# esteinig/sketchy

Hardware: AMD Instinct MI355X
Metric: reads/sec streamed (s=10000,k=16,40k-genome ref) (higher is better)
Workload: dtype u64

## Files before the change

### sketchy_amd/csrc/skx_capi.hip

```cpp
#include <dlfcn.h>
#include <hip/hip_runtime.h>
#include <rccl/rccl.h>

#include <unistd.h>

#include <algorithm>
#include <atomic>
#include <chrono>
#include <cmath>
#include <condition_variable>
#include <cstdarg>
#include <cstdio>
#include <cstdlib>
#include <cstring>
#include <mutex>
#include <string>
#include <thread>
#include <unordered_map>
#include <vector>

#include "sketchy_hip.h"
#include "skx_common.hpp"
#include "skx_kernels.hpp"

// ... 914 lines not shown
    bool back_pending[2] = {false, false};
    hipEvent_t ev_pslot[3] = {nullptr, nullptr, nullptr};
    bool pslot_pending[3] = {false, false, false};
    int pslot = 0;
    hipEvent_t ev_pairq[2] = {nullptr, nullptr};
    bool pairq_pending[2] = {false, false};
    bool packed = false;
    u32 top_k = 0, max_reads = 0, sk_stride = 0;
    u64 max_bases = 0;
    u32 pcap = 0;
    u32 qcap = 0;
    u64* d_qd = nullptr;
    u32 *d_qrow = nullptr, *d_sslot = nullptr, *d_qinfo = nullptr, *d_qloc = nullptr, *d_cls_bsum = nullptr;
    u32* d_nd_hs = nullptr;
    u32* h_lcount = nullptr;
    u32 lcount_seq = 0, lcount_seen = 0, lcount_floor = 0;
    u32* h_nq_sink = nullptr;
    u32* h_nd = nullptr;
    u32 *d_rowcnt = nullptr;
    u32 *d_gain = nullptr;
    u32 *d_gain_s = nullptr;
    u32 *d_candslot = nullptr;
    u32 *d_candmask = nullptr;
    uint2 *d_lrow = nullptr;
    u32 *d_nlrow = nullptr, *d_gain_l = nullptr, *d_cbase = nullptr, *d_cwl = nullptr, *d_ncwl = nullptr;
    u64 *d_cw = nullptr;
    u64 *d_inb = nullptr, *d_hit = nullptr;
    skx::LongRows long_rows() const { return skx::LongRows{d_lrow, d_nlrow, qcap + 128, d_inb, ref->n_lw}; }
    bool use_pat = false;
    u32 *d_hist = nullptr, *d_nprow = nullptr;
    u64* d_pcw = nullptr;
    u32 npat_pad = 0;
    skx::PatRows pat_rows() const { return skx::PatRows{d_hist, npat_pad, d_gain_l, d_nprow}; }
    skx::RareIndex rare_index() const {
        skx::RareIndex ri = ref->rare_index();
        if (!use_pat) { ri.prec = nullptr; ri.n_pat = 0; }
        if (!static_dense) { ri.qs = nullptr; ri.n_sd = 0; }
        return ri;
    }
    u32 *d_cbad = nullptr, *d_nqc = nullptr;
    u32 *d_spc_g0 = nullptr, *d_spc_grp = nullptr;
    u32 n_pad_c = 0, n_grp_c = 0, cand_seq = 0;
    struct PassSet {
        u64 *tab = nullptr;
        u32 *cand = nullptr;
        u64 *tabc = nullptr;
        u32 *ncand = nullptr;
        u32 *mode = nullptr, *any_full = nullptr, *nqc_total = nullptr;
        u64 *mc = nullptr;
        u64 *mqc = nullptr;
        u64 *rowany_c = nullptr;
        u32 *grp_any_c = nullptr;
        u32 *smap = nullptr;
        u32 *pair_qc = nullptr;
        u32 *nd = nullptr;
        u32 *h_pub = nullptr;
    } ps[2];
    struct PassChains {
        bool pending = false, ranked = false, has_cand = false, update_table = false, forced_full = false, legacy = false;
        SubPass subs[kGroupMax];
        int n_sub = 0, b = 0, slot = 0;
        u32 P = 0, nq_rows = 0, seq = 0;
        u64 nq_est = 0;
    } pcq[2];
    int pc_head = 0, pc_n = 0;
    bool hint_all_overflow = false;
    u32 hint_seq = 0;
    u32 passes_since_fresh = 0;
    bool fresh_table = true;
    u32 legacy_run = 0;
    u64 batches_compact = 0, batches_full = 0;
    bool have_split_hint = false;
    double nd_frac = 1.0;
    u32 qcap_max = 0;
    bool qcap_auto = false;
    u64 qrows_grown = 0;
    u32 coalesce = 1;
    u32 rpass = 0;
    u64 reads_total = 0;
    uint8_t* d_bases = nullptr;
    u64* d_offsets = nullptr;
    u64* d_sk = nullptr;
    u32 *d_len = nullptr, *d_cnt = nullptr, *d_poff = nullptr;
    bool side_ready[kSides] = {};
    u64* sd_sk[kSides] = {};
    u64 pool_cap[kSides] = {};
    u32 pool_fixed = 0;
    u64* sd_rows[kSides] = {};
    u32 cur_stride = 0;
    u32 cur_pool_cap = 0, cur_pool_fixed = 0;
    u32 *sd_len[kSides] = {}, *sd_cnt[kSides] = {}, *sd_poff[kSides] = {}, *sd_big[kSides] = {};
// ... 130 lines not shown
static void free_side(skx_stream* st, int i);
static void free_lane(skx_stream* st, int i);
static void free_call(CallOut& d) {
    void* ptrs[] = {d.sp, d.idx, d.sum, d.codes, d.n_events, d.ev_read, d.ev_sp, d.ev_idx, d.ev_sum, d.ev_codes};
    for (void* q : ptrs) (void)hipFree(q);
    d = CallOut{};
}
static void stream_free(skx_stream* st) {
    if (!st) return;
    (void)hipSetDevice(st->device);
    if (st->hs0) (void)hipStreamSynchronize(st->hs0);
    if (st->hs1) (void)hipStreamSynchronize(st->hs1);
    if (st->hs) (void)hipStreamSynchronize(st->hs);
    if (st->hs2) (void)hipStreamSynchronize(st->hs2);
    for (int i = 1; i < skx_stream::kRankLanes; ++i)
        if (st->lane[i].s) (void)hipStreamSynchronize(st->lane[i].s);
    for (int i = 0; i < kSides; ++i) (void)hipFree(st->sd_rows[i]);
    void* ptrs[] = {st->d_bases, st->d_offsets, st->d_pair_h[0], st->d_pair_h[1],
                    st->d_q[0], st->d_q[1], st->d_pair_r[0], st->d_pair_r[1], st->d_pair_q[0], st->d_pair_q[1],
                    st->d_poff_pass[0], st->d_poff_pass[1], st->d_poff_pass[2], st->d_pair_r[2], st->d_nq[0], st->d_nq[1], st->d_win[0], st->d_win[1], st->d_m, st->d_mint, st->d_mq[0], st->d_mq[1],
                    st->d_topk_idx, st->d_topk_sum, st->d_cons, st->d_ev.n_events, st->d_ev.ev_read, st->d_ev.ev_idx, st->d_ev.ev_sum, st->d_ev.ev_codes, st->d_tab_tmp, st->d_rank_idx, st->d_rank_sum, st->d_bsum, st->d_grp_any[0],
                    st->d_grp_any[1], st->d_hbuf, st->d_wb[0], st->d_wb[1], st->d_rowany[0], st->d_rowany[1], st->d_mqext,
                    st->d_qd, st->d_qrow, st->d_sslot, st->d_qinfo, st->d_qloc, st->d_cls_bsum, st->d_nd_hs,
                    st->d_rowcnt, st->d_gain, st->d_gain_s, st->d_candslot, st->d_candmask, st->d_lrow, st->d_nlrow, st->d_gain_l, st->d_cbase, st->d_cwl, st->d_ncwl, st->d_cw, st->d_cbad, st->d_nqc, st->d_spc_g0, st->d_spc_grp, st->d_inb, st->d_hit, st->d_hist, st->d_nprow, st->d_pcw, st->d_ms[0], st->d_ms[1], st->d_mdirty_s};
    for (auto& q : st->ps) {
        for (void* x : {(void*)q.tab, (void*)q.cand, (void*)q.tabc, (void*)q.ncand, (void*)q.mode, (void*)q.any_full, (void*)q.nqc_total, (void*)q.mc, (void*)q.mqc,
                        (void*)q.rowany_c, (void*)q.grp_any_c, (void*)q.smap, (void*)q.pair_qc, (void*)q.nd}) (void)hipFree(x);
        if (q.h_pub) (void)hipHostFree(q.h_pub);
    }
    for (auto& t : st->d_tab) (void)hipFree(t);
    for (int i = 0; i < skx_stream::kRankLanes; ++i) free_lane(st, i);
    for (int i = 1; i < skx_stream::kRankLanes; ++i)
        if (st->own_lane_stream && st->lane[i].s) (void)hipStreamDestroy(st->lane[i].s);
    for (void* p : ptrs) (void)hipFree(p);
    for (void* p : {(void*)st->d_seen, (void*)st->d_cov_pad, (void*)st->d_cov_out, (void*)st->d_cov_list, (void*)st->d_cov_ridx,
                    (void*)st->d_cov_wide, (void*)st->d_cov_rsum}) (void)hipFree(p);
    if (st->h_poff) (void)hipHostFree(st->h_poff);
    if (st->h_offsets) (void)hipHostFree(st->h_offsets);
    if (st->h_nq) (void)hipHostFree(st->h_nq);
    if (st->h_nd) (void)hipHostFree(st->h_nd);
    if (st->h_nq_sink) (void)hipHostFree(st->h_nq_sink);
    if (st->h_lcount) (void)hipHostFree(st->h_lcount);
    if (st->h_chk_base) (void)hipHostFree(st->h_chk_base);
    for (int i = 0; i < kSides; ++i) {
        free_side(st, i);
        if (st->ev_main[i]) (void)hipEventDestroy(st->ev_main[i]);
    }
// ... 398 lines not shown
    memset(st->h_nd, 0, 4 * 4);
    SCHK(hipHostMalloc((void**)&st->h_nq_sink, 4 * 4, hipHostMallocCoherent));
    SCHK(hipHostMalloc((void**)&st->h_lcount, 4 * 4, hipHostMallocCoherent));
    memset(st->h_lcount, 0, 4 * 4);
    SCHK(hipMalloc(&st->d_nd_hs, 64));
    SCHK(hipMemset(st->d_nd_hs, 0, 64));
    if (ref->d_kt_key) {
        SCHK(hipMalloc(&st->d_qd, (size_t)st->pcap * 8));
        SCHK(hipMalloc(&st->d_qrow, (size_t)st->pcap * 4));
        SCHK(hipMalloc(&st->d_sslot, (size_t)st->pcap * 8));
        SCHK(hipMalloc(&st->d_qinfo, (size_t)st->pcap * 4));
        SCHK(hipMalloc(&st->d_qloc, (size_t)st->pcap * 4));
        SCHK(hipMalloc(&st->d_cls_bsum, ((size_t)st->pcap / 1024 + 2) * 4));
    }
    {
        const u32 nb = skx::kPassBatchesMax, cap = skx::kCandCap, rows_c = skx::kCandRows;
        st->n_pad_c = n_sp * cap;
        st->n_grp_c = st->n_pad_c / (skx::kRankWords * 64);
        SCHK(hipMalloc(&st->d_rowcnt, (size_t)nb * ((size_t)st->qcap + 128) * 4));
        SCHK(hipMalloc(&st->d_gain, (size_t)nb * n_pad * 4));
        if (ref->d_kt_key) SCHK(hipMalloc(&st->d_gain_s, (size_t)nb * n_pad * 4 * skx::gain_sparse_stride()));
        SCHK(hipMalloc(&st->d_candslot, (size_t)nb * n_pad * 4));
        SCHK(hipMalloc(&st->d_candmask, (size_t)n_pad * 4));
        if (ref->d_mlong) {
            SCHK(hipMalloc(&st->d_lrow, (size_t)nb * ((size_t)st->qcap + 128) * 8));
            SCHK(hipMalloc(&st->d_nlrow, skx::pass_counter_bytes()));
            SCHK(hipMalloc(&st->d_gain_l, (size_t)nb * n_pad * 4));
            SCHK(hipMalloc(&st->d_cw, (size_t)nb * (n_pad / 64) * 8));
            SCHK(hipMalloc(&st->d_cbase, (size_t)nb * (n_pad / 64) * 4));
            SCHK(hipMalloc(&st->d_cwl, (size_t)nb * st->n_pad_c * 4));
            SCHK(hipMalloc(&st->d_ncwl, 64));
            if (ref->d_mlongT) {
                SCHK(hipMalloc(&st->d_inb, (size_t)nb * ref->n_lw * 8));
                SCHK(hipMalloc(&st->d_hit, (size_t)nb * ref->n_lw * 8));
            }
            if (ref->d_prec && ref->n_pat && st->n_grp_c * skx::kRankWords <= skx::pat_words_max()) {
                st->use_pat = true;
                st->npat_pad = (ref->n_pat + 63u) & ~63u;
                SCHK(hipMalloc(&st->d_hist, (size_t)nb * st->npat_pad * 4));
                SCHK(hipMalloc(&st->d_nprow, skx::pass_counter_bytes()));
                SCHK(hipMalloc(&st->d_pcw, (size_t)nb * ref->n_pat * st->n_grp_c * skx::kRankWords * 8));
            }
        }
        SCHK(hipMalloc(&st->d_cbad, 64));
        SCHK(hipMalloc(&st->d_nqc, skx::pass_counter_bytes()));
        std::vector<u32> g0c(n_sp), grpc(st->n_grp_c);
// ... 296 lines not shown
    HIPCHK(hipMemsetAsync(d_mdirty, 0, 4, hs));
    SKX_MARK("pass: memset mdirty", 0);
    auto wait_back = [&]() -> int {
        if (st->back_pending[b]) { HIPCHK(hipStreamWaitEvent(hs, st->ev_back[b], 0)); st->back_pending[b] = false; }
        HIPCHK(hipMemcpyAsync(ps.nd, d_nd, 16, hipMemcpyDeviceToDevice, hs));
        HIPCHK(hipMemsetAsync(d_grp_any, 0, (size_t)n_grp_all * 4, hs));
        if (P > 0) {
            skx::launch_pair_q(hs, st->d_pair_h[b], P, d_q, d_nq, d_pair_q, split_dict ? st->d_qrow : nullptr, st->d_bbase, st->d_btot, ref->max_ref);
            HIPCHK(hipGetLastError());
        }
        HIPCHK(hipEventRecord(st->ev_pairq[b], hs));
        st->pairq_pending[b] = true;
        return SKX_OK;
    };
    bool ranked = false, all_forced = false, all_ranked = true;
    for (int i = 0; i < n_sub; ++i) {
        const bool r = st->top_k && subs[i].d_topk_idx && subs[i].d_topk_sum;
        ranked = ranked || r; all_ranked = all_ranked && r && !subs[i].d_shared && !subs[i].d_counts;
    }
    const u32* only_if = nullptr;
    u32 seq = 0;
    static const int legacy_env = skx::knob("SKX_TABLE_LEGACY") ? atoi(skx::knob("SKX_TABLE_LEGACY")) : 1 << 30;
    static const int cand_env0 = skx::knob("SKX_CAND") ? atoi(skx::knob("SKX_CAND")) : 1;
    const bool fresh_overflow = st->fresh_table && ref->max_species > skx::kCandCap && st->top_k <= 1;
    const bool second_blind = st->passes_since_fresh == 1 && !((int)(st->lcount_seen - st->lcount_floor) > 0);
    const bool legacy = update_table && all_ranked && cand_env0 && legacy_env > 0 &&
                        (fresh_overflow || (st->hint_all_overflow && !second_blind && (int)st->legacy_run < legacy_env));
    st->legacy_run = legacy ? st->legacy_run + 1 : 0;
    if (update_table) { st->passes_since_fresh = st->fresh_table ? 1 : st->passes_since_fresh + 1; st->fresh_table = false; }
    const bool long_rows = split_dict && ref->d_mlong != nullptr;
    static const int tail_env = skx::knob("SKX_TAIL_SCALE") ? atoi(skx::knob("SKX_TAIL_SCALE")) : 8;
    const u32 walk_scale = st->tail_pass ? (u32)std::max(1, tail_env) : 1u;
    skx::PassBatches pbt;
    pbt.n = (u32)n_sub;
    for (int i = 0; i < n_sub; ++i) pbt.p_off[i] = subs[i].p_off;
    pbt.p_off[n_sub] = P;
    auto rare_gains = [&](hipStream_t on) -> int {
        const skx::RareIndex ri = st->rare_index();
        const skx::LongRows lrows = st->long_rows();
        const skx::PatRows prows = st->pat_rows();
        skx::launch_gain_sparse(on, d_nd, q_bound, st->d_rowcnt, qstride, (u32)n_sub, n_pad, st->d_gain_s, st->d_sslot, ri, long_rows ? &lrows : nullptr, walk_scale,
                                (long_rows && st->use_pat) ? &prows : nullptr);
        if (long_rows) skx::launch_gain_long(on, lrows, ri, d_nd, st->d_rowcnt, qstride, (u32)n_sub, n_pad, st->d_gain_l, walk_scale);
        if (long_rows && st->use_pat)
            skx::launch_gain_dense(on, ri.pm, nullptr, n_pad, ri.d_npat, ri.n_pat, st->d_hist, st->npat_pad, (u32)n_sub, st->d_gain_l);
        HIPCHK(hipGetLastError());
        return SKX_OK;
    };
    auto row_counts = [&]() -> int {
        HIPCHK(hipMemset2DAsync(st->d_rowcnt, (size_t)qstride * 4, 0, (size_t)nq_rows * 4, (size_t)n_sub, hs));
        skx::launch_pass_hist(hs, d_pair_q, pbt, st->d_rowcnt, qstride);
        if (split_dict) HIPCHK(hipMemsetAsync(st->d_gain_s, 0, (size_t)n_sub * n_pad * 4 * skx::gain_sparse_stride(), hs));
// ... 61 lines not shown
        const u64* m_int = split ? st->d_mint : nullptr;
        HIPCHK(hipMemsetAsync(st->d_gain, 0, (size_t)n_sub * n_pad * 4, hs));
        if (P > 0) {
            SKXCHK(row_counts());
            skx::launch_gain_dense(hs, d_m, m_int, n_pad, d_nd, sdm ? ref->n_sd : q_bound, st->d_rowcnt, qstride, (u32)n_sub, st->d_gain,
                                   (sdm && ref->n_species > 1) ? ref->d_segw : nullptr, ref->d_grp_sp);
            if (split_dict) SKXCHK(rare_gains(hs));
        }
        skx::launch_pass_tables(hs, st->d_cum, st->d_gain, (split_dict && P > 0) ? st->d_gain_s : nullptr,
                                (long_rows && P > 0) ? st->d_gain_l : nullptr, (u32)n_sub, n_pad, ps.tab);
        st->d_cum = ps.tab + (size_t)n_sub * n_pad;
        static const int cand_env = skx::knob("SKX_CAND") ? atoi(skx::knob("SKX_CAND")) : 1;
        static const int hint_env = skx::knob("SKX_CAND_HINT") ? atoi(skx::knob("SKX_CAND_HINT")) : 1;
        (void)hint_env;
        all_forced = !cand_env;
        u32 force_full = all_forced ? 0xFFu : 0u;
        for (int i = 0; i < n_sub; ++i) if (subs[i].d_shared || subs[i].d_counts) force_full |= 1u << i;
        HIPCHK(hipMemsetAsync(st->d_cbad, 0, 64, hs));
        HIPCHK(hipMemsetAsync(st->d_nqc, 0, skx::pass_counter_bytes(), hs));
        const bool pat_rows = st->use_pat && long_rows && ranked && P > 0 && !all_forced;
        if (pat_rows) skx::launch_pat_nqc_init(hs, st->d_nqc, st->npat_pad);
        if (ranked) {
            HIPCHK(hipMemsetAsync(st->d_candmask, 0, (size_t)n_pad * 4, hs));
            skx::launch_cand_select(hs, ps.tab, n_pad, spc, (u32)n_sub, st->top_k, cap, ps.cand, st->d_candslot, ps.tabc, ps.ncand, st->d_cbad,
                                    st->d_candmask);
            HIPCHK(hipMemsetAsync(ps.grp_any_c, 0, (size_t)n_sub * st->n_grp_c * 4, hs));
            if (split_dict && P > 0 && !all_forced) {
                HIPCHK(hipMemsetAsync(ps.mqc, 0, (size_t)n_sub * st->n_grp_c * rows_c * skx::kRankWords * 8, hs));
                HIPCHK(hipMemsetAsync(ps.rowany_c, 0, (size_t)n_sub * st->n_grp_c * (rows_c / 64) * 8, hs));
                HIPCHK(hipMemset2DAsync(ps.smap, (size_t)qstride * 4, 0, (size_t)nq_rows * 4, (size_t)n_sub, hs));
                skx::launch_cand_sparse(hs, st->d_sslot, d_nd, q_bound, st->rare_index(), st->d_candmask, st->d_candslot, n_pad, st->d_cbad, (u32)n_sub, st->d_nqc,
                                        ps.smap, qstride, ps.mqc, (size_t)st->n_grp_c * rows_c * skx::kRankWords, rows_c, ps.rowany_c,
                                        st->n_grp_c * (rows_c / 64), ps.grp_any_c, st->n_grp_c, walk_scale);
                if (long_rows) {
                    const u32 n_gw = n_pad / 64;
                    HIPCHK(hipMemsetAsync(st->d_cw, 0, (size_t)n_sub * n_gw * 8, hs));
                    HIPCHK(hipMemsetAsync(st->d_cbase, 0xFF, (size_t)n_sub * n_gw * 4, hs));
                    HIPCHK(hipMemsetAsync(st->d_ncwl, 0, 64, hs));
                    skx::launch_cand_words(hs, ps.cand, st->n_pad_c, (u32)n_sub, n_gw, st->d_cw, st->d_cbase, st->d_cwl, st->d_ncwl);
                    if (st->d_hit) skx::launch_cand_hit(hs, ps.cand, st->n_pad_c, (u32)n_sub, st->d_cbad, st->rare_index(), st->d_inb, st->d_hit);
                    skx::launch_cand_long(hs, st->long_rows(), st->rare_index(), d_nd, st->d_cw, st->d_cbase, st->d_cwl, st->d_ncwl, st->n_pad_c,
                                          st->d_cbad, (u32)n_sub, st->d_nqc, ps.smap, qstride, ps.mqc, (size_t)st->n_grp_c * rows_c * skx::kRankWords,
                                          rows_c, ps.rowany_c, st->n_grp_c * (rows_c / 64), ps.grp_any_c, st->n_grp_c, walk_scale, st->d_hit);
                }
                if (pat_rows) {
                    const skx::RareIndex ri = st->rare_index();
                    skx::launch_cand_pat_rows(hs, ri, d_nd, st->d_candmask, st->d_candslot, n_pad, st->d_cbad, (u32)n_sub, st->d_pcw, ps.mqc,
                                              (size_t)st->n_grp_c * rows_c * skx::kRankWords, rows_c, ps.rowany_c, st->n_grp_c * (rows_c / 64), ps.grp_any_c,
// ... 373 lines not shown
    if (call) sb.call = *call;
    sb.ra = ra; sb.rb = rb; sb.p_off = 0; sb.P = P; sb.p_base = p_base; sb.d_topk_idx = d_topk_idx; sb.d_topk_sum = d_topk_sum;
    sb.d_shared = d_shared; sb.d_counts = d_counts; sb.side = st->side;
    sb.d_poff = st->d_poff_pass[st->pslot];
    return run_pass_multi(st, &sb, 1, update_table, inserted, q_rows);
}

template <class F>
static int for_each_pass(skx_stream* st, u32 n_reads, u32 max_pass_reads, F fn) {
    const u32 cap = std::max<u32>(1u, std::min<u32>(st->rpass, max_pass_reads));
    const u32 pair_cap = std::min(st->pcap, st->qhash_cap());
    u32 ra = 0;
    while (ra < n_reads) {
        u32 rb = ra;
        while (rb < n_reads && rb - ra < cap && st->h_poff[rb + 1] - st->h_poff[ra] <= pair_cap) ++rb;
        if (rb == ra) return fail(SKX_ERR_CAPACITY, "read %u alone has %u candidate hashes > pass capacity %u", ra,
                                  st->h_poff[ra + 1] - st->h_poff[ra], pair_cap);
        SKXCHK(fn(ra, rb, st->h_poff[ra], st->h_poff[rb] - st->h_poff[ra]));
        ra = rb;
    }
    return SKX_OK;
}

static int wait_published(skx_stream* st, const PendingBatch& pb) {
    volatile u32* pub = st->h_chk_base + 16 * pb.side;
    hipStream_t hs = st->hs1;
    for (u64 spins = 1; pub[15] != pb.seq; ++spins) {
        if ((spins & 0xFFF) == 0) {
            const hipError_t e = hipStreamQuery(hs);
            if (e == hipSuccess) {
                if (pub[15] == pb.seq) break;
                HIPCHK(hipStreamSynchronize(hs));
                if (pub[15] != pb.seq) return fail(SKX_ERR_HIP, "publish kernel finished without raising its sequence number");
            } else if (e != hipErrorNotReady) {
                return fail(SKX_ERR_HIP, "stream failed while waiting for the batch summary: %s", hipGetErrorString(e));
            }
        }
    }
    return SKX_OK;
}
static const u64* batch_filter(const skx_ref* ref) {
    static const bool no_filter = skx::knob("SKX_NO_FILTER") != nullptr;
    return (ref->any && !no_filter) ? ref->d_filt : nullptr;
}
static int behind_the_sketch(skx_stream* st, int side) {
    if (st->hs1 == st->hs0) return SKX_OK;
    HIPCHK(hipEventRecord(st->ev_main[side], st->hs0));
    HIPCHK(hipStreamWaitEvent(st->hs1, st->ev_main[side], 0));
    return SKX_OK;
}
// ... 279 lines not shown
    }
    SKX_ACC(back);
#ifdef SKX_EXPERIMENTS
    g_ht.n += 1;
    if (skx::knob("SKX_HOST_TIMES") && (g_ht.n % 64) == 0)
        fprintf(stderr, "[skx host times] per batch over %llu: front %.1f us, wait for summary %.1f us, queue passes %.1f us\n",
                (unsigned long long)g_ht.n, g_ht.front / g_ht.n, g_ht.wait / g_ht.n, g_ht.back / g_ht.n);
#endif
    if (d_shared) (void)hipFree(d_shared);
    SKXCHK(pass_rc);
    st->reads_total += n_reads;
    return SKX_OK;
}

static int batch_back_group(skx_stream* st, PendingBatch* g, int n, PendingBatch* younger, int* n_done) {
    *n_done = 0;
    if (n == 1) {
        SKXCHK(batch_back(st, g[0], younger));
        *n_done = 1;
        return SKX_OK;
    }
    {
        SKX_T0();
        for (int i = 0; i < n; ++i) SKXCHK(wait_published(st, g[i]));
        SKX_ACC(wait);
    }
    bool fits = st->buf == g[0].spec_set && st->pslot == g[0].spec_slot;
    u64 pairs = 0;
    u32 P[kGroupMax];
    for (int i = 0; i < n; ++i) {
        const volatile u32* c = st->h_chk_base + 16 * g[i].side;
        fits = fits && !(c[0] | c[6] | c[7]);
        P[i] = c[8];
        pairs += P[i];
    }
    const u32 q_rows = (st->h_chk_base + 16 * g[n - 1].side)[10];
    const bool clean = fits;
    if (clean && q_rows != 0xFFFFFFFFu && q_rows > st->qhash_cap() && pairs <= st->pcap)
        SKXCHK(grow_query_rows(st, ((u64)q_rows + q_rows / 4) * std::max<u32>(1u, (st->coalesce + (u32)n - 1) / (u32)n)));
    fits = fits && pairs <= st->pcap && q_rows != 0xFFFFFFFFu && q_rows <= st->qhash_cap();
    u64 reads = 0;
    for (int i = 0; i < n; ++i) reads += g[i].n_reads;
    if (clean && q_rows != 0xFFFFFFFFu && reads) {
        st->ppr_est = (double)pairs / reads;
        st->qpr_est = (double)q_rows / reads;
    }
    if (clean && !fits) {
// ... 1738 lines not shown
```

### sketchy_amd/csrc/skx_kernels.hip

```cpp
#include <algorithm>
#include <cstdlib>
#include <mutex>
#include <type_traits>

#include "skx_common.hpp"
#include "skx_kernels.hpp"

#ifndef SKX_FEW_CANDS
#define SKX_FEW_CANDS 8
#endif
#ifndef SKX_SCAN_ROWS
#define SKX_SCAN_ROWS 8
#endif
#ifndef SKX_SCAN_OCC
#define SKX_SCAN_OCC 1
#endif
#ifndef SKX_SCAN_SPLIT_READS
#define SKX_SCAN_SPLIT_READS 1
#endif
#ifndef SKX_WALK_BLOCKS
#define SKX_WALK_BLOCKS 256
#endif
#ifndef SKX_GAIN_SPARSE_STRIDE
#define SKX_GAIN_SPARSE_STRIDE 16
// ... 4200 lines not shown
    return theta;
}
__global__ __launch_bounds__(1024) void cand_count_kernel(const u64* __restrict__ t0, const u64* __restrict__ t1, Species sp, u32 top_k,
                                                          u32* __restrict__ d_max, volatile u32* __restrict__ h_out, u32 seq) {
    __builtin_amdgcn_s_setprio(3);
    __shared__ u64 sh64[16];
    __shared__ u32 sh32[16];
    u32 worst = 0;
    for (u32 spi = 0; spi < sp.n_sp; ++spi) {
        const u32 g0 = sp.g0[spi], n = sp.n[spi];
        const u64 theta = species_theta(t0, g0, n, top_k, sh64, sh32);
        u32 c = 0;
        for (u32 g = g0 + threadIdx.x; g < g0 + n; g += 1024u) c += t1[g] >= theta ? 1u : 0u;
        worst = max(worst, block1024_sum_u32(c, sh32));
    }
    if (threadIdx.x == 0u) {
        (void)d_max;
        h_out[0] = worst;
        __threadfence_system();
        h_out[1] = seq;
        __threadfence_system();
    }
}
__global__ __launch_bounds__(1024) void cand_select_kernel(const u64* __restrict__ tab, u32 n_pad, Species sp, u32 top_k, u32 cap,
                                                           u32* __restrict__ cand, u32* __restrict__ candslot, u64* __restrict__ tabc,
                                                           u32* __restrict__ ncand, u32* __restrict__ bad, u32* __restrict__ candmask) {
    __builtin_amdgcn_s_setprio(3);
    __shared__ u64 sh64[16];
    __shared__ u32 sh32[16];
    __shared__ u32 wbase[17];
    const u32 b = blockIdx.x / sp.n_sp, spi = blockIdx.x % sp.n_sp, tid = threadIdx.x, lane = lane_id(), wv = tid >> 6;
    const u32 g0 = sp.g0[spi], n = sp.n[spi];
    const u32 g_end = spi + 1u < sp.n_sp ? sp.g0[spi + 1u] : n_pad;
    const u64* t0 = tab + (size_t)b * n_pad;
    const u64* t1 = t0 + n_pad;
    const u64 theta = species_theta(t0, g0, n, top_k, sh64, sh32);
    u32 base = 0;
    u32* my_cand = cand + (size_t)(b * sp.n_sp + spi) * cap;
    u64* my_tabc = tabc + (size_t)b * sp.n_sp * cap + (size_t)spi * cap;
    for (u32 c0 = g0; c0 < g_end; c0 += 1024u) {
        const u32 g = c0 + tid;
        const bool is = g < g0 + n && t1[g] >= theta;
        const u64 bal = __ballot(is);
        const u32 before = (u32)__popcll(bal & lanemask_lt()), wtot = (u32)__popcll(bal);
        __syncthreads();
        if (lane == 0u) wbase[wv] = wtot;
        __syncthreads();
        u32 wb = 0, tot = 0;
#pragma unroll
        for (u32 i = 0; i < 16u; ++i) { const u32 v = wbase[i]; wb += i < wv ? v : 0u; tot += v; }
        const u32 pos = base + wb + before;
        if (g < g_end) {
            u32 slot = kCandNone;
            if (is && pos < cap) { my_cand[pos] = g; my_tabc[pos] = t0[g]; slot = spi * cap + pos; atomicOr(&candmask[g], 1u << b); }
            candslot[(size_t)b * n_pad + g] = slot;
        }
        base += tot;
    }
    for (u32 i = min(base, cap) + tid; i < cap; i += 1024u) { my_cand[i] = kCandNone; my_tabc[i] = 0; }
    if (tid == 0u) {
        ncand[b * sp.n_sp + spi] = min(base, cap);
        if (base > cap) atomicOr(&bad[b], 1u);
    }
}
__global__ __launch_bounds__(256) void cand_gather_m_kernel(const u64* __restrict__ m_bits, const u64* __restrict__ m_int, u32 n_pad,
                                                            const u32* __restrict__ n_d,
                                                            const u32* __restrict__ cand, u32 n_pad_c, const u32* __restrict__ bad,
                                                            u64* __restrict__ mc, u32 words_c) {
    __builtin_amdgcn_s_setprio(2);
    const u32 b = blockIdx.z, w = blockIdx.y, c = blockIdx.x * 256u + threadIdx.x;
    if (bad[b] || w >= ((n_d[0] + 63u) >> 6) || c >= n_pad_c) return;
    const u32 g = cand[(size_t)b * n_pad_c + c];
    u64 x = 0;
    if (g != kCandNone) { x = m_bits[(size_t)w * n_pad + g]; if (m_int) x |= m_int[(size_t)w * n_pad + g]; }
    mc[((size_t)b * words_c + w) * n_pad_c + c] = x;
}
__global__ __launch_bounds__(256) void cand_sparse_kernel(const u32* __restrict__ sslot, const u32* __restrict__ n_d, RareIndex ri,
                                                          const u32* __restrict__ candmask, const u32* __restrict__ candslot, u32 n_pad,
                                                          u32* __restrict__ bad, u32 n_b, u32* __restrict__ nqc, u32* __restrict__ smap,
                                                          u32 smap_stride, u64* __restrict__ mqc, size_t mqc_stride, u32 rows_c,
                                                          u64* __restrict__ rowany_c, u32 rowany_stride, u32* __restrict__ grp_any_c,
                                                          u32 n_grp_c) {
    __builtin_amdgcn_s_setprio(2);
    __shared__ u64 pat[4][kPassBatchesMax][kPatWords];
    const u32 nd64 = n_d[2], ns = n_d[1], lane = lane_id();
    const u32 n_gw_c = n_grp_c * kRankWords;
    const u32 wave = blockIdx.x * 4u + (threadIdx.x >> 6), n_waves = gridDim.x * 4u;
    auto put = [&](u32 b, u32 crow, u32 slot) { atomicOr(&mqc[(size_t)b * mqc_stride + mq_index(slot >> 6, crow, rows_c)], 1ull << (slot & 63u)); };
    auto flag = [&](u32 b, u32 crow, u32 grp) {
        atomicOr(&rowany_c[(size_t)b * rowany_stride + (size_t)grp * (rows_c >> 6) + (crow >> 6)], 1ull << (crow & 63u));
        u32* ga = grp_any_c + (size_t)b * n_grp_c + grp;
        if (*ga == 0u) atomicOr(ga, 1u);
    };
    auto new_row = [&](u32 b, u32 sr) -> u32 {
        if (bad[b]) return kCandNone;
        const u32 crow = nd64 + atomicAdd(&nqc[b * kCtrStride], 1u);
        if (crow + 1u >= rows_c) { atomicOr(&bad[b], 2u); return kCandNone; }
        smap[(size_t)b * smap_stride + sr] = crow + 1u;
        return crow;
    };
    for (u32 r0 = wave * 64u; r0 < ns; r0 += n_waves * 64u) {
        const u32 sr = r0 + lane;
        u32 off = 0, np = 0;
        if (sr < ns) { const uint2 e = reinterpret_cast<const uint2*>(sslot)[sr]; off = e.x; np = e.y; }
        if (np & kLongFlag) np = 0;
        if (np && np <= 8u) {
            u32 crow[kPassBatchesMax];
#pragma unroll
            for (u32 b = 0; b < kPassBatchesMax; ++b) crow[b] = kCandNone;
            for (u32 j = 0; j < np; ++j) {
// ... 554 lines not shown
                      u32* gain_l, u32 walk_scale) {
    hipLaunchKernelGGL(gain_long_kernel, dim3(cdiv(ri.n_gw, 64), n_b, (u32)env_int("SKX_G_GAINLONG", 8) * std::min(4u, std::max(1u, walk_scale))), dim3(256), 0, st, lr, ri, n_d, cnt, row_stride, n_pad, gain_l);
}
void launch_mlong_transpose(hipStream_t st, const u64* mlong, u32 n_long, u32 n_gw, u64* mlongT, u32 n_lw) {
    if (n_long == 0) return;
    hipLaunchKernelGGL(mlong_transpose_kernel, dim3(n_lw, cdiv(n_gw, 4)), dim3(256), 0, st, mlong, n_long, n_gw, mlongT, n_lw);
}
void launch_cand_hit(hipStream_t st, const u32* cand, u32 n_pad_c, u32 n_b, const u32* bad, const RareIndex& ri, const u64* inb, u64* hit) {
    hipLaunchKernelGGL(cand_hit_kernel, dim3(cdiv(n_pad_c, 4), n_b), dim3(256), 0, st, cand, n_pad_c, bad, ri, inb, hit);
}
void launch_cand_words(hipStream_t st, const u32* cand, u32 n_pad_c, u32 n_b, u32 n_gw, u64* cw, u32* cbase, u32* cwl, u32* ncwl) {
    hipLaunchKernelGGL(cand_words_kernel, dim3(n_b), dim3(1024), 0, st, cand, n_pad_c, n_gw, cw, cbase, cwl, ncwl);
}
void launch_cand_long(hipStream_t st, const LongRows& lr, const RareIndex& ri, const u32* n_d, const u64* cw, const u32* cbase, const u32* cwl,
                      const u32* ncwl, u32 n_pad_c, u32* bad, u32 n_b, u32* nqc, u32* smap, u32 smap_stride, u64* mqc, size_t mqc_stride,
                      u32 rows_c, u64* rowany_c, u32 rowany_stride, u32* grp_any_c, u32 n_grp_c, u32 walk_scale, const u64* hit) {
    hipLaunchKernelGGL(cand_long_kernel, dim3((u32)env_int("SKX_G_CANDLONG", 192) * std::min(4u, std::max(1u, walk_scale)), n_b), dim3(256), 0, st, lr, ri, n_d, cw, cbase, cwl, ncwl, n_pad_c, bad, nqc, smap, smap_stride, mqc,
                       mqc_stride, rows_c, rowany_c, rowany_stride, grp_any_c, n_grp_c, hit);
}
void launch_pass_tables(hipStream_t st, const u64* prev, const u32* gain, const u32* gain_s, const u32* gain_l, u32 n_b, u32 n_pad, u64* tab) {
    hipLaunchKernelGGL(pass_tables_kernel, dim3(cdiv(n_pad, 256)), dim3(256), 0, st, prev, gain, gain_s, gain_l, n_b, n_pad, tab);
}
void launch_cand_select(hipStream_t st, const u64* tab, u32 n_pad, const Species& sp, u32 n_b, u32 top_k, u32 cap, u32* cand, u32* candslot,
                        u64* tabc, u32* ncand, u32* bad, u32* candmask) {
    hipLaunchKernelGGL(cand_select_kernel, dim3(n_b * sp.n_sp), dim3(1024), 0, st, tab, n_pad, sp, top_k, cap, cand, candslot, tabc, ncand, bad, candmask);
}
void launch_cand_count(hipStream_t st, const u64* t0, const u64* t1, const Species& sp, u32 top_k, u32* h_out, u32 seq) {
    hipLaunchKernelGGL(cand_count_kernel, dim3(1), dim3(1024), 0, st, t0, t1, sp, top_k, nullptr, h_out, seq);
}
void launch_cand_gather_m(hipStream_t st, const u64* m_bits, const u64* m_int, u32 n_pad, const u32* n_d, u32 rows_bound, const u32* cand, u32 n_pad_c,
                          const u32* bad, u32 n_b, u64* mc, u32 words_c) {
    const u32 words = std::min(words_c, std::max(1u, cdiv(rows_bound, 64)));
    hipLaunchKernelGGL(cand_gather_m_kernel, dim3(cdiv(n_pad_c, 256), words, n_b), dim3(256), 0, st, m_bits, m_int, n_pad, n_d, cand, n_pad_c, bad, mc, words_c);
}
void launch_cand_sparse(hipStream_t st, const u32* sslot, const u32* n_d, u32 rows_bound, const RareIndex& ri, const u32* candmask,
                        const u32* candslot, u32 n_pad, u32* bad, u32 n_b, u32* nqc, u32* smap, u32 smap_stride, u64* mqc, size_t mqc_stride,
                        u32 rows_c, u64* rowany_c, u32 rowany_stride, u32* grp_any_c, u32 n_grp_c, u32 walk_scale) {
    hipLaunchKernelGGL(cand_sparse_kernel, dim3(std::max(1u, std::min(cdiv(rows_bound, 256), kWalkBlocks * std::max(1u, walk_scale)))), dim3(256), 0, st, sslot, n_d, ri, candmask,
                       candslot, n_pad, bad, n_b, nqc, smap, smap_stride, mqc, mqc_stride, rows_c, rowany_c, rowany_stride, grp_any_c, n_grp_c);
}
void launch_cand_publish(hipStream_t st, const u32* bad, u32 force_full, const u32* ncand, const u32* nqc, const u32* n_d, u32 n_b, u32 n_sp,
                         u32 rows_c, u32* mode, u32* any_full, u32* nqc_total, u32* h_pub, u32 seq) {
    hipLaunchKernelGGL(cand_publish_kernel, dim3(1), dim3(1), 0, st, bad, force_full, ncand, nqc, n_d, n_b, n_sp, rows_c, mode, any_full, nqc_total,
                       h_pub, seq);
}
void launch_m_clear(hipStream_t st, u64* m_bits, u64* m_int, u32 n_pad, const u32* n_d, const u32* any_full) {
    hipLaunchKernelGGL(m_clear_kernel, dim3(512), dim3(256), 0, st, m_bits, m_int, n_pad, n_d, any_full);
}
// ... 701 lines not shown
```

### sketchy_amd/csrc/skx_kernels.hpp

```cpp
#pragma once
#include <hip/hip_runtime.h>
#include <stddef.h>
#include <stdint.h>

#include <stdlib.h>

namespace skx {
typedef unsigned long long u64;
typedef unsigned int u32;

inline const char* knob(const char* name) {
#ifdef SKX_EXPERIMENTS
    return getenv(name);
#else
    (void)name;
    return nullptr;
#endif
}

constexpr int kSketchCap = 2048;
constexpr u32 kSegLen = 64;
constexpr int kRankWords = 8;

struct Species { const u32* g0; const u32* n; const u32* of_grp; u32 n_sp; };
// ... 70 lines not shown
                        u32 rows_bound, const u32* only_if = nullptr );
void launch_nd_from_nq(hipStream_t st, const u32* n_q, u32* n_d, u32* h_words);

static const u32 kPassBatchesMax = 8;
static const u32 kCandCap = 1024;
static const u32 kCandRows = 131072;
struct PassBatches { u32 n; u32 p_off[kPassBatchesMax + 1]; };
void launch_pass_hist(hipStream_t st, const u32* pair_q, const PassBatches& pb, u32* cnt, u32 row_stride);
void launch_gain_dense(hipStream_t st, const u64* m_bits, const u64* m_int , u32 n_pad, const u32* n_d, u32 rows_bound, const u32* cnt,
                       u32 row_stride, u32 n_b, u32* gain, const u32* segw = nullptr ,
                       const u32* grp_sp = nullptr);
void launch_gain_sparse(hipStream_t st, const u32* n_d, u32 rows_bound, const u32* cnt, u32 row_stride, u32 n_b, u32 n_pad, u32* gain_s,
                        const u32* sslot, const RareIndex& ri, const LongRows* lr, u32 walk_scale, const PatRows* pr = nullptr);
void launch_pat_nqc_init(hipStream_t st, u32* nqc, u32 v);
void launch_cand_pat_rows(hipStream_t st, const RareIndex& ri, const u32* n_d, const u32* candmask, const u32* candslot, u32 n_pad, u32* bad, u32 n_b,
                          u64* pcw, u64* mqc, size_t mqc_stride, u32 rows_c, u64* rowany_c, u32 rowany_stride, u32* grp_any_c, u32 n_grp_c);
void launch_cand_pat_map(hipStream_t st, const LongRows& lr, const PatRows& pr, const RareIndex& ri, const u32* n_d, const u32* candmask,
                         const u32* candslot, u32 n_pad, u32* bad, u32 n_b, u32* nqc, u32* smap, u32 smap_stride, const u64* pcw, u64* mqc,
                         size_t mqc_stride, u32 rows_c, u64* rowany_c, u32 rowany_stride, u32* grp_any_c, u32 n_grp_c, u32 rows_bound, u32 walk_scale = 1);
u32 gain_sparse_stride();
void launch_pass_tables(hipStream_t st, const u64* prev, const u32* gain, const u32* gain_s , const u32* gain_l , u32 n_b,
                        u32 n_pad, u64* tab);
void launch_cand_select(hipStream_t st, const u64* tab, u32 n_pad, const Species& sp, u32 n_b, u32 top_k, u32 cap, u32* cand, u32* candslot,
                        u64* tabc, u32* ncand, u32* bad, u32* candmask);
void launch_cand_count(hipStream_t st, const u64* t0, const u64* t1, const Species& sp, u32 top_k, u32* h_out, u32 seq);
void launch_cand_gather_m(hipStream_t st, const u64* m_bits, const u64* m_int , u32 n_pad, const u32* n_d, u32 rows_bound, const u32* cand,
                          u32 n_pad_c, const u32* bad, u32 n_b, u64* mc, u32 words_c);
void launch_cand_sparse(hipStream_t st, const u32* sslot, const u32* n_d, u32 rows_bound, const RareIndex& ri, const u32* candmask,
                        const u32* candslot, u32 n_pad, u32* bad, u32 n_b, u32* nqc, u32* smap, u32 smap_stride, u64* mqc, size_t mqc_stride,
                        u32 rows_c, u64* rowany_c, u32 rowany_stride, u32* grp_any_c, u32 n_grp_c, u32 walk_scale = 1);
void launch_cand_publish(hipStream_t st, const u32* bad, u32 force_full, const u32* ncand, const u32* nqc, const u32* n_d, u32 n_b, u32 n_sp,
                         u32 rows_c, u32* mode, u32* any_full, u32* nqc_total, u32* h_pub, u32 seq);
void launch_m_clear(hipStream_t st, u64* m_bits, u64* m_int , u32 n_pad, const u32* n_d, const u32* any_full);
void launch_cand_pair_rows(hipStream_t st, const u32* pair_q, u32 n_pairs, const u32* n_d, const u32* smap, u32 rows_c, u32* pair_qc);
void launch_cand_rows_back(hipStream_t st, u32* out_idx, u32 n_reads, u32 n_sp, u32 top_k, const u32* cand, u32 cap, const u32* g0);
constexpr u32 kConsensusTopMax = 64;
void launch_consensus_rows(hipStream_t st, const u32* idx, u64 first_row, u64 n_rows, u32 n_sp, u32 top_k, const u32* g0, const u32* codes,
                           u32 n_feat, u32* out, u32 n_code_rows);
constexpr u32 kChangeWidthMax = 4096;
void launch_change_flags(hipStream_t st, const u32* rows, u32 width, u32 ra, u32 rb, u32* flag);
void launch_change_events(hipStream_t st, const u32* flag, u32* pos, u32* bsum, u32 n, u32 cap, u32* n_events, u32* ev_read,
                          const u32* idx, const u64* sum, u32 w_idx, u32* ev_idx, u64* ev_sum, const u32* codes, u32 w_codes, u32* ev_codes);
void launch_species_call(hipStream_t st, const u32* idx, const u64* sum, const u32* codes, u32 ra, u32 rb, u32 n_sp, u32 top_k, u32 n_feat,
                         u32* call_sp, u32* call_idx, u64* call_sum, u32* call_codes, u32* key, bool key_codes);
void launch_call_species_gather(hipStream_t st, const u32* flag, const u32* pos, u32 n, u32 cap, const u32* call_sp, u32* ev_sp);

void launch_pair_q(hipStream_t st, const u64* pair_h, u32 n_pairs, const u64* q, const u32* n_q, u32* pair_q, const u32* qrow ,
// ... 112 lines not shown
```

Measured before the change: 150.3 million.

## Prune overflowing candidate sets with a leader-masked upper-bound gain

For single-species top-1 runs, a new kernel finds each batch's current leader and flags batches whose candidate count exceeds the cap. A masked gain kernel then computes, per genome, the gain only over rows the leader has not yet covered. Candidate selection uses this as a tighter bound, so fewer genomes qualify and fewer passes fall back to the costly legacy full-table path. It also adds an early exit in candidate mapping when every batch is already marked bad, and polls queued chains while waiting for publication. The cost is extra kernels, memsets and buffers, plus more involved legacy-decision state.

After: 143.3 million. -4.6%, worse.

```diff
diff --git a/sketchy_amd/csrc/skx_capi.hip b/sketchy_amd/csrc/skx_capi.hip
--- a/sketchy_amd/csrc/skx_capi.hip
+++ b/sketchy_amd/csrc/skx_capi.hip
@@ -960,6 +960,8 @@
     u32 *d_gain_s = nullptr;
     u32 *d_candslot = nullptr;
     u32 *d_candmask = nullptr;
+    u32 *d_ugain = nullptr;
+    u32 *d_lead = nullptr, *d_need = nullptr;
     uint2 *d_lrow = nullptr;
     u32 *d_nlrow = nullptr, *d_gain_l = nullptr, *d_cbase = nullptr, *d_cwl = nullptr, *d_ncwl = nullptr;
     u64 *d_cw = nullptr;
@@ -1005,6 +1007,7 @@
     bool hint_all_overflow = false;
     u32 hint_seq = 0;
     u32 passes_since_fresh = 0;
+    bool fresh_legacy = true;
     bool fresh_table = true;
     u32 legacy_run = 0;
     u64 batches_compact = 0, batches_full = 0;
@@ -1181,7 +1184,7 @@
                     st->d_topk_idx, st->d_topk_sum, st->d_cons, st->d_ev.n_events, st->d_ev.ev_read, st->d_ev.ev_idx, st->d_ev.ev_sum, st->d_ev.ev_codes, st->d_tab_tmp, st->d_rank_idx, st->d_rank_sum, st->d_bsum, st->d_grp_any[0],
                     st->d_grp_any[1], st->d_hbuf, st->d_wb[0], st->d_wb[1], st->d_rowany[0], st->d_rowany[1], st->d_mqext,
                     st->d_qd, st->d_qrow, st->d_sslot, st->d_qinfo, st->d_qloc, st->d_cls_bsum, st->d_nd_hs,
-                    st->d_rowcnt, st->d_gain, st->d_gain_s, st->d_candslot, st->d_candmask, st->d_lrow, st->d_nlrow, st->d_gain_l, st->d_cbase, st->d_cwl, st->d_ncwl, st->d_cw, st->d_cbad, st->d_nqc, st->d_spc_g0, st->d_spc_grp, st->d_inb, st->d_hit, st->d_hist, st->d_nprow, st->d_pcw, st->d_ms[0], st->d_ms[1], st->d_mdirty_s};
+                    st->d_rowcnt, st->d_gain, st->d_gain_s, st->d_candslot, st->d_candmask, st->d_ugain, st->d_lead, st->d_need, st->d_lrow, st->d_nlrow, st->d_gain_l, st->d_cbase, st->d_cwl, st->d_ncwl, st->d_cw, st->d_cbad, st->d_nqc, st->d_spc_g0, st->d_spc_grp, st->d_inb, st->d_hit, st->d_hist, st->d_nprow, st->d_pcw, st->d_ms[0], st->d_ms[1], st->d_mdirty_s};
     for (auto& q : st->ps) {
         for (void* x : {(void*)q.tab, (void*)q.cand, (void*)q.tabc, (void*)q.ncand, (void*)q.mode, (void*)q.any_full, (void*)q.nqc_total, (void*)q.mc, (void*)q.mqc,
                         (void*)q.rowany_c, (void*)q.grp_any_c, (void*)q.smap, (void*)q.pair_qc, (void*)q.nd}) (void)hipFree(x);
@@ -1626,6 +1629,11 @@
         if (ref->d_kt_key) SCHK(hipMalloc(&st->d_gain_s, (size_t)nb * n_pad * 4 * skx::gain_sparse_stride()));
         SCHK(hipMalloc(&st->d_candslot, (size_t)nb * n_pad * 4));
         SCHK(hipMalloc(&st->d_candmask, (size_t)n_pad * 4));
+        if (n_sp == 1 && top_k == 1) {
+            SCHK(hipMalloc(&st->d_ugain, (size_t)nb * n_pad * 4));
+            SCHK(hipMalloc(&st->d_lead, (size_t)nb * 4));
+            SCHK(hipMalloc(&st->d_need, (size_t)skx::cand_need_words() * 4));
+        }
         if (ref->d_mlong) {
             SCHK(hipMalloc(&st->d_lrow, (size_t)nb * ((size_t)st->qcap + 128) * 8));
             SCHK(hipMalloc(&st->d_nlrow, skx::pass_counter_bytes()));
@@ -1968,12 +1976,16 @@
     u32 seq = 0;
     static const int legacy_env = skx::knob("SKX_TABLE_LEGACY") ? atoi(skx::knob("SKX_TABLE_LEGACY")) : 1 << 30;
     static const int cand_env0 = skx::knob("SKX_CAND") ? atoi(skx::knob("SKX_CAND")) : 1;
-    const bool fresh_overflow = st->fresh_table && ref->max_species > skx::kCandCap && st->top_k <= 1;
-    const bool second_blind = st->passes_since_fresh == 1 && !((int)(st->lcount_seen - st->lcount_floor) > 0);
+    const bool leader_rule = st->d_need != nullptr;
+    const bool fresh_overflow = st->fresh_table && ref->max_species > skx::kCandCap && st->top_k <= 1 && (!leader_rule || n_sub == 1);
+    const bool second_blind = st->passes_since_fresh == 1 && st->fresh_legacy && !((int)(st->lcount_seen - st->lcount_floor) > 0);
     const bool legacy = update_table && all_ranked && cand_env0 && legacy_env > 0 &&
                         (fresh_overflow || (st->hint_all_overflow && !second_blind && (int)st->legacy_run < legacy_env));
     st->legacy_run = legacy ? st->legacy_run + 1 : 0;
-    if (update_table) { st->passes_since_fresh = st->fresh_table ? 1 : st->passes_since_fresh + 1; st->fresh_table = false; }
+    if (update_table) {
+        if (st->fresh_table || st->passes_since_fresh == 0) st->fresh_legacy = legacy;
+        st->passes_since_fresh = st->fresh_table ? 1 : st->passes_since_fresh + 1; st->fresh_table = false;
+    }
     const bool long_rows = split_dict && ref->d_mlong != nullptr;
     static const int tail_env = skx::knob("SKX_TAIL_SCALE") ? atoi(skx::knob("SKX_TAIL_SCALE")) : 8;
     const u32 walk_scale = st->tail_pass ? (u32)std::max(1, tail_env) : 1u;
@@ -2081,8 +2093,17 @@
         if (pat_rows) skx::launch_pat_nqc_init(hs, st->d_nqc, st->npat_pad);
         if (ranked) {
             HIPCHK(hipMemsetAsync(st->d_candmask, 0, (size_t)n_pad * 4, hs));
+            const bool by_leader = leader_rule && P > 0 && !all_forced && m_int == nullptr;
+            if (by_leader) {
+                HIPCHK(hipMemsetAsync(st->d_need, 0, (size_t)skx::cand_need_words() * 4, hs));
+                HIPCHK(hipMemsetAsync(st->d_ugain, 0, (size_t)n_sub * n_pad * 4, hs));
+                skx::launch_cand_leader(hs, ps.tab, n_pad, spc, (u32)n_sub, cap, st->d_lead, st->d_need);
+                skx::launch_gain_masked(hs, d_m, n_pad, d_nd, sdm ? ref->n_sd : q_bound, st->d_rowcnt, qstride, (u32)n_sub, st->d_lead, st->d_need,
+                                        st->d_ugain);
+            }
             skx::launch_cand_select(hs, ps.tab, n_pad, spc, (u32)n_sub, st->top_k, cap, ps.cand, st->d_candslot, ps.tabc, ps.ncand, st->d_cbad,
-                                    st->d_candmask);
+                                    st->d_candmask, by_leader ? st->d_need : nullptr, st->d_ugain, split_dict ? st->d_gain_s : nullptr,
+                                    long_rows ? st->d_gain_l : nullptr);
             HIPCHK(hipMemsetAsync(ps.grp_any_c, 0, (size_t)n_sub * st->n_grp_c * 4, hs));
             if (split_dict && P > 0 && !all_forced) {
                 HIPCHK(hipMemsetAsync(ps.mqc, 0, (size_t)n_sub * st->n_grp_c * rows_c * skx::kRankWords * 8, hs));
@@ -2502,10 +2523,11 @@
     return SKX_OK;
 }
 
-static int wait_published(skx_stream* st, const PendingBatch& pb) {
+static int wait_published(skx_stream* st, const PendingBatch& pb, bool poll_chains = false) {
     volatile u32* pub = st->h_chk_base + 16 * pb.side;
     hipStream_t hs = st->hs1;
     for (u64 spins = 1; pub[15] != pb.seq; ++spins) {
+        if (poll_chains && (spins & 0xFF) == 0 && st->pc_n > 0) SKXCHK(queue_chains(st, false));
         if ((spins & 0xFFF) == 0) {
             const hipError_t e = hipStreamQuery(hs);
             if (e == hipSuccess) {
@@ -2831,7 +2853,7 @@
     }
     {
         SKX_T0();
-        for (int i = 0; i < n; ++i) SKXCHK(wait_published(st, g[i]));
+        for (int i = 0; i < n; ++i) SKXCHK(wait_published(st, g[i], true));
         SKX_ACC(wait);
     }
     bool fits = st->buf == g[0].spec_set && st->pslot == g[0].spec_slot;
diff --git a/sketchy_amd/csrc/skx_kernels.hip b/sketchy_amd/csrc/skx_kernels.hip
--- a/sketchy_amd/csrc/skx_kernels.hip
+++ b/sketchy_amd/csrc/skx_kernels.hip
@@ -4246,9 +4246,73 @@
         __threadfence_system();
     }
 }
+__global__ __launch_bounds__(1024) void cand_leader_kernel(const u64* __restrict__ tab, u32 n_pad, Species sp, u32 cap,
+                                                           u32* __restrict__ leader, u32* __restrict__ need) {
+    __builtin_amdgcn_s_setprio(3);
+    __shared__ u64 sh64[16];
+    __shared__ u32 sh32[16];
+    const u32 b = blockIdx.x, g0 = sp.g0[0], n = sp.n[0];
+    const u64* t0 = tab + (size_t)b * n_pad;
+    const u64* t1 = t0 + n_pad;
+    u64 m = 0;
+    for (u32 g = g0 + threadIdx.x; g < g0 + n; g += 1024u) m = max(m, t0[g]);
+    m = block1024_max_u64(m, sh64);
+    u32 c = 0, first = 0xFFFFFFFFu;
+    for (u32 g = g0 + threadIdx.x; g < g0 + n; g += 1024u) {
+        c += t1[g] >= m ? 1u : 0u;
+        if (t0[g] == m) first = min(first, g);
+    }
+    c = block1024_sum_u32(c, sh32);
+    first = ~(u32)block1024_max_u64((u64)(~first), sh64);
+    if (threadIdx.x == 0u) {
+        leader[b] = first;
+        if (c > cap && first != 0xFFFFFFFFu) { need[b] = 1u; atomicOr(&need[kPassBatchesMax], 1u); }
+    }
+}
+template <u32 NB>
+__global__ __launch_bounds__(256) void gain_masked_kernel(const u64* __restrict__ m_bits, u32 n_pad, const u32* __restrict__ n_d,
+                                                          const u32* __restrict__ cnt, u32 row_stride, const u32* __restrict__ leader,
+                                                          const u32* __restrict__ need, u32* __restrict__ ugain) {
+    __builtin_amdgcn_s_setprio(2);
+    if (need[kPassBatchesMax] == 0u) return;
+    const u32 g = blockIdx.x * 256u + threadIdx.x;
+    const u32 nd = n_d[0], n_words = (nd + 63u) >> 6;
+    const u32 w0 = blockIdx.y * kGainWords;
+    if (w0 >= n_words) return;
+    const u32 w1 = min(n_words, w0 + kGainWords);
+    u32 acc[NB], lead[NB];
+#pragma unroll
+    for (u32 b = 0; b < NB; ++b) { acc[b] = 0; lead[b] = need[b] ? leader[b] : 0xFFFFFFFFu; }
+    for (u32 w = w0; w < w1; ++w) {
+        const u32 rows = min(64u, nd - w * 64u);
+        u64 open[NB], open_any = 0;
+#pragma unroll
+        for (u32 b = 0; b < NB; ++b) {
+            open[b] = lead[b] != 0xFFFFFFFFu ? ~m_bits[(size_t)w * n_pad + lead[b]] : 0ull;
+            if (rows < 64u) open[b] &= (1ull << rows) - 1ull;
+            open_any |= open[b];
+        }
+        if (open_any == 0ull) continue;
+        const u64 m = m_bits[(size_t)w * n_pad + g];
+        if (__ballot((m & open_any) != 0ull) == 0ull) continue;
+        const u32 lo = (u32)m, hi = (u32)(m >> 32);
+        const u32* c = cnt + (size_t)w * 64u;
+        for (u64 rem = open_any; rem != 0ull; rem &= rem - 1ull) {
+            const u32 j = (u32)__builtin_ctzll(rem);
+            const u32 bit = j < 32u ? __builtin_amdgcn_ubfe(lo, j, 1u) : __builtin_amdgcn_ubfe(hi, j - 32u, 1u);
+#pragma unroll
+            for (u32 b = 0; b < NB; ++b) acc[b] += __umul24(bit, ((open[b] >> j) & 1ull) ? c[(size_t)b * row_stride + j] : 0u);
+        }
+    }
+#pragma unroll
+    for (u32 b = 0; b < NB; ++b)
+        if (acc[b]) atomicAdd(&ugain[(size_t)b * n_pad + g], acc[b]);
+}
 __global__ __launch_bounds__(1024) void cand_select_kernel(const u64* __restrict__ tab, u32 n_pad, Species sp, u32 top_k, u32 cap,
                                                            u32* __restrict__ cand, u32* __restrict__ candslot, u64* __restrict__ tabc,
-                                                           u32* __restrict__ ncand, u32* __restrict__ bad, u32* __restrict__ candmask) {
+                                                           u32* __restrict__ ncand, u32* __restrict__ bad, u32* __restrict__ candmask,
+                                                           const u32* __restrict__ need, const u32* __restrict__ ugain,
+                                                           const u32* __restrict__ gain_s, const u32* __restrict__ gain_l) {
     __builtin_amdgcn_s_setprio(3);
     __shared__ u64 sh64[16];
     __shared__ u32 sh32[16];
@@ -4259,12 +4323,20 @@
     const u64* t0 = tab + (size_t)b * n_pad;
     const u64* t1 = t0 + n_pad;
     const u64 theta = species_theta(t0, g0, n, top_k, sh64, sh32);
+    const bool by_leader = need != nullptr && need[b] != 0u;
     u32 base = 0;
     u32* my_cand = cand + (size_t)(b * sp.n_sp + spi) * cap;
     u64* my_tabc = tabc + (size_t)b * sp.n_sp * cap + (size_t)spi * cap;
     for (u32 c0 = g0; c0 < g_end; c0 += 1024u) {
         const u32 g = c0 + tid;
-        const bool is = g < g0 + n && t1[g] >= theta;
+        bool is = g < g0 + n && t1[g] >= theta;
+        if (by_leader && is) {
+            const size_t i = (size_t)b * n_pad + g;
+            u64 u = ugain[i];
+            if (gain_s) u += gain_s[i * kGainSparseStride];
+            if (gain_l) u += gain_l[i];
+            is = t0[g] + u >= theta;
+        }
         const u64 bal = __ballot(is);
         const u32 before = (u32)__popcll(bal & lanemask_lt()), wtot = (u32)__popcll(bal);
         __syncthreads();
@@ -4310,6 +4382,11 @@
     const u32 nd64 = n_d[2], ns = n_d[1], lane = lane_id();
     const u32 n_gw_c = n_grp_c * kRankWords;
     const u32 wave = blockIdx.x * 4u + (threadIdx.x >> 6), n_waves = gridDim.x * 4u;
+    {
+        u32 open = 0;
+        for (u32 b = 0; b < n_b; ++b) open |= bad[b] == 0u ? 1u : 0u;
+        if (!open) return;
+    }
     auto put = [&](u32 b, u32 crow, u32 slot) { atomicOr(&mqc[(size_t)b * mqc_stride + mq_index(slot >> 6, crow, rows_c)], 1ull << (slot & 63u)); };
     auto flag = [&](u32 b, u32 crow, u32 grp) {
         atomicOr(&rowany_c[(size_t)b * rowany_stride + (size_t)grp * (rows_c >> 6) + (crow >> 6)], 1ull << (crow & 63u));
@@ -4910,8 +4987,24 @@
     hipLaunchKernelGGL(pass_tables_kernel, dim3(cdiv(n_pad, 256)), dim3(256), 0, st, prev, gain, gain_s, gain_l, n_b, n_pad, tab);
 }
 void launch_cand_select(hipStream_t st, const u64* tab, u32 n_pad, const Species& sp, u32 n_b, u32 top_k, u32 cap, u32* cand, u32* candslot,
-                        u64* tabc, u32* ncand, u32* bad, u32* candmask) {
-    hipLaunchKernelGGL(cand_select_kernel, dim3(n_b * sp.n_sp), dim3(1024), 0, st, tab, n_pad, sp, top_k, cap, cand, candslot, tabc, ncand, bad, candmask);
+                        u64* tabc, u32* ncand, u32* bad, u32* candmask, const u32* need, const u32* ugain, const u32* gain_s, const u32* gain_l) {
+    if (top_k != 1 || sp.n_sp != 1) need = nullptr;
+    hipLaunchKernelGGL(cand_select_kernel, dim3(n_b * sp.n_sp), dim3(1024), 0, st, tab, n_pad, sp, top_k, cap, cand, candslot, tabc, ncand, bad, candmask,
+                       need, ugain, gain_s, gain_l);
+}
+u32 cand_need_words() { return kPassBatchesMax + 1u; }
+void launch_cand_leader(hipStream_t st, const u64* tab, u32 n_pad, const Species& sp, u32 n_b, u32 cap, u32* leader, u32* need) {
+    hipLaunchKernelGGL(cand_leader_kernel, dim3(n_b), dim3(1024), 0, st, tab, n_pad, sp, cap, leader, need);
+}
+void launch_gain_masked(hipStream_t st, const u64* m_bits, u32 n_pad, const u32* n_d, u32 rows_bound, const u32* cnt, u32 row_stride, u32 n_b,
+                        const u32* leader, const u32* need, u32* ugain) {
+    const dim3 grid(n_pad / 256, std::max(1u, cdiv(cdiv(rows_bound, 64), kGainWords)));
+#define SKX_GAINM(NB) hipLaunchKernelGGL(gain_masked_kernel<NB>, grid, dim3(256), 0, st, m_bits, n_pad, n_d, cnt, row_stride, leader, need, ugain)
+    switch (n_b) {
+        case 1: SKX_GAINM(1); break; case 2: SKX_GAINM(2); break; case 3: SKX_GAINM(3); break; case 4: SKX_GAINM(4); break;
+        case 5: SKX_GAINM(5); break; case 6: SKX_GAINM(6); break; case 7: SKX_GAINM(7); break; default: SKX_GAINM(8); break;
+    }
+#undef SKX_GAINM
 }
 void launch_cand_count(hipStream_t st, const u64* t0, const u64* t1, const Species& sp, u32 top_k, u32* h_out, u32 seq) {
     hipLaunchKernelGGL(cand_count_kernel, dim3(1), dim3(1024), 0, st, t0, t1, sp, top_k, nullptr, h_out, seq);
diff --git a/sketchy_amd/csrc/skx_kernels.hpp b/sketchy_amd/csrc/skx_kernels.hpp
--- a/sketchy_amd/csrc/skx_kernels.hpp
+++ b/sketchy_amd/csrc/skx_kernels.hpp
@@ -116,7 +116,12 @@
 void launch_pass_tables(hipStream_t st, const u64* prev, const u32* gain, const u32* gain_s , const u32* gain_l , u32 n_b,
                         u32 n_pad, u64* tab);
 void launch_cand_select(hipStream_t st, const u64* tab, u32 n_pad, const Species& sp, u32 n_b, u32 top_k, u32 cap, u32* cand, u32* candslot,
-                        u64* tabc, u32* ncand, u32* bad, u32* candmask);
+                        u64* tabc, u32* ncand, u32* bad, u32* candmask, const u32* need = nullptr, const u32* ugain = nullptr,
+                        const u32* gain_s = nullptr, const u32* gain_l = nullptr);
+u32 cand_need_words();
+void launch_cand_leader(hipStream_t st, const u64* tab, u32 n_pad, const Species& sp, u32 n_b, u32 cap, u32* leader, u32* need);
+void launch_gain_masked(hipStream_t st, const u64* m_bits, u32 n_pad, const u32* n_d, u32 rows_bound, const u32* cnt, u32 row_stride, u32 n_b,
+                        const u32* leader, const u32* need, u32* ugain);
 void launch_cand_count(hipStream_t st, const u64* t0, const u64* t1, const Species& sp, u32 top_k, u32* h_out, u32 seq);
 void launch_cand_gather_m(hipStream_t st, const u64* m_bits, const u64* m_int , u32 n_pad, const u32* n_d, u32 rows_bound, const u32* cand,
                           u32 n_pad_c, const u32* bad, u32 n_b, u64* mc, u32 words_c);
```
